# eikehmueller/mlmcpathintegral

Hardware: AMD Instinct MI355X
Metric: lattice-site-updates/sec (higher is better)
Workload: dtype f64

## Files before the change

mlmcpathintegral_amd/csrc/schwinger_perm.hpp:

```cpp
#pragma once
#include "lattice_sweep.hpp"

namespace mlmcpi {

#ifdef MLMCPI_STAMPS
__device__ unsigned long long g_stamps[16 * 65536];
#define MLMCPI_STAMP(k)                                                                                            \
  do {                                                                                                             \
    if (threadIdx.x == 0 && blockIdx.y * gridDim.x + blockIdx.x < 65536)                                           \
      g_stamps[(blockIdx.y * gridDim.x + blockIdx.x) * 16 + (k)] = __builtin_amdgcn_s_memrealtime();               \
  } while (0)
#define MLMCPI_STAMP_WHERE()                                                                                       \
  do {                                                                                                             \
    if (threadIdx.x == 0 && blockIdx.y * gridDim.x + blockIdx.x < 65536)                                           \
      g_stamps[(blockIdx.y * gridDim.x + blockIdx.x) * 16 + 15] =                                                  \
          ((unsigned long long)__builtin_amdgcn_s_getreg((20 ) | (0 << 6) | (31 << 11)) << 32) |         \
          __builtin_amdgcn_s_getreg((4 ) | (0 << 6) | (31 << 11));                                        \
  } while (0)
#else
#define MLMCPI_STAMP(k) do { } while (0)
#define MLMCPI_STAMP_WHERE() do { } while (0)
#endif

#ifndef MLMCPI_PERM_U
#define MLMCPI_PERM_U 0
#endif

template <class PG>
struct PermPlane {
  static constexpr int kRow = PG::kPitch * 8, kStep = kRow + 8;
  static constexpr uint32_t QB = (uint32_t)PG::kQRows * kRow;
  static_assert(kStep == (int)PG::kStep * 8, "the stride of a stream");
  uint32_t K;
  __device__ __forceinline__ explicit PermPlane(uint32_t K_) : K(K_) {}
  __device__ __forceinline__ bool has_col(uint32_t C) const { return (C & 1u) ? C <= PG::col_last(K, 1) : C >= PG::col_first(K, 0) && C <= PG::col_last(K, 0); }
  __device__ __forceinline__ bool has_row(uint32_t R) const { return (R & 1u) ? R <= PG::row_last(K, 1) : R >= PG::row_first(K, 0) && R <= PG::row_last(K, 0); }
  __device__ __forceinline__ uint32_t col(uint32_t C) const { return (C & 1u) ? QB + PG::col_u(K, C) * 8u : PG::col_u(K, C) * 8u; }
  __device__ __forceinline__ uint32_t row(uint32_t R) const { return (R & 1u) ? 2u * QB + PG::row_v(K, R) * (uint32_t)kRow : PG::row_v(K, R) * (uint32_t)kRow; }
};

struct PermBuildPos {
  uint32_t c, r, rend, row_off, gj;
  uint32_t cb;
  const double2 *src;
  uint32_t col;
  bool active, owns;
};
template <int NT, class PP>
__device__ __forceinline__ PermBuildPos perm_build_pos(const PP &P, const double2 *__restrict__ src, uint32_t Mt, uint32_t Mx, uint32_t gi0,
                                                       uint32_t gj0, uint32_t W, uint32_t rows) {
  PermBuildPos q;
  const uint32_t wave = __builtin_amdgcn_readfirstlane(threadIdx.x / kWave), lane = threadIdx.x % kWave;
  const uint32_t nwc = W > 63 ? 2 : 1;
  const uint32_t groups = (NT / kWave) >> (nwc - 1);
  const uint32_t g = wave >> (nwc - 1), cw = wave & (nwc - 1);
  static_assert(((NT / kWave) & (NT / kWave - 1)) == 0, "waves per workgroup: a power of two (shifts for divisions)");
  const uint32_t rpg = groups == 4 ? (rows + 3) >> 2 : groups == 8 ? (rows + 7) >> 3 : (rows + groups - 1) / groups;
  q.c = 63 * cw + lane;
  q.r = __builtin_amdgcn_readfirstlane(g * rpg);
  q.rend = __builtin_amdgcn_readfirstlane(g < groups ? min(rows, q.r + rpg) : 0);
  q.active = q.r < q.rend;
  q.owns = lane < 63 && q.c < W && P.has_col(q.c);
  q.cb = P.col(q.c);
  q.src = src;
  q.col = wrap_add(gi0, min(q.c, W), Mt);
  q.gj = __builtin_amdgcn_readfirstlane(wrap_add(gj0, q.r, Mx));
  q.row_off = q.gj * Mt;
  return q;
}
template <int U>
__device__ __forceinline__ void perm_rows_load(PermBuildPos &q, uint32_t Mt, uint32_t Mx, bool first, double2 &cur, double2 (&nxt)[U]) {
  if (!q.active) return;
  if (first) cur = (q.src + q.row_off)[q.col];
#pragma unroll
  for (int u = 0; u < U; ++u) {
    q.gj = q.gj + 1 == Mx ? 0 : q.gj + 1;
    q.row_off = q.gj == 0 ? 0 : q.row_off + Mt;
    if (q.r + u < q.rend) nxt[u] = (q.src + q.row_off)[q.col];
  }
}
template <int U, class PP>
__device__ __forceinline__ void perm_rows_store(PermBuildPos &q, const PP &P, double *plane, double2 &cur, const double2 (&nxt)[U]) {
  if (!q.active) return;
  char *const pb = reinterpret_cast<char *>(plane) + q.cb;
#pragma unroll
  for (int u = 0; u < U; ++u)
    if (q.r + u < q.rend) {
      const double right = wave_rotate_down(cur.y);
      if (q.owns && P.has_row(q.r + u)) *reinterpret_cast<double *>(pb + P.row(q.r + u)) = ((cur.x + right) - nxt[u].x) - cur.y;
      cur = nxt[u];
    }
  q.r += U;
}
template <int NT, int U, bool ONCE, class PP>
__device__ __forceinline__ void perm_build_rows(const PP &P, double *plane, const double2 *__restrict__ src, uint32_t Mt, uint32_t Mx,
                                                uint32_t gi0, uint32_t gj0, uint32_t W, uint32_t rows) {
  PermBuildPos q = perm_build_pos<NT>(P, src, Mt, Mx, gi0, gj0, W, rows);
  double2 cur = make_double2(0., 0.);
  if (ONCE) {
    double2 nxt[U];
    perm_rows_load<U>(q, Mt, Mx, true, cur, nxt);
    perm_rows_store<U>(q, P, plane, cur, nxt);
    return;
  }
  bool first = true;
  while (__builtin_amdgcn_readfirstlane(q.r) < __builtin_amdgcn_readfirstlane(q.rend)) {
    double2 nxt[U];
    perm_rows_load<U>(q, Mt, Mx, first, cur, nxt);
    perm_rows_store<U>(q, P, plane, cur, nxt);
    first = false;
  }
}

template <int NT, int RING, int TH = 64>
struct PermTasks {
  using PG = PermGeom<NT, RING, TH>;
  static constexpr int OW = PG::OW, HR = PG::HR, H2 = HR / 2, NW = NT / kWave, NS = (HR + NW - 1) / NW;
  static constexpr int XC = OW - 64;
  static constexpr int L0 = XC * H2, L1 = (XC / 2) * HR;
  static constexpr int NL0 = (L0 + 63) / 64, NL1 = (L1 + 63) / 64;
  static constexpr int WF = HR - NW * (NS - 1);
  static_assert(PG::NV == NS, "slots per thread");
  static_assert(NL0 + NL1 <= NW - WF, "the left-over wave-tasks fit the free last slots");
  uint32_t wave, lane, c_mu0, c_mu1, r_lo;
  __device__ PermTasks() {
    wave = __builtin_amdgcn_readfirstlane(threadIdx.x / kWave);
    lane = threadIdx.x % kWave;
    c_mu0 = lane < 32 ? 2 * lane : 2 * (lane - 32) + 1;
    c_mu1 = 2 * (lane & 31u);
    r_lo = lane >> 5;
  }
  __device__ __forceinline__ bool task(int k, bool &mu1, uint32_t &r, uint32_t &c) const {
    const uint32_t m = wave + (uint32_t)(NW * k);
    mu1 = false; r = 0; c = 0;
    if (NW * k + NW - 1 < H2 || m < (uint32_t)H2) {
      r = 2 * m;
      c = c_mu0;
      return true;
    }
    if (m < (uint32_t)HR) {
      mu1 = true;
      r = 2 * (m - H2) + r_lo;
      c = c_mu1;
      return true;
    }
    if (XC > 0 && k == NS - 1) {
      const uint32_t j = wave - (uint32_t)WF;
      if (j < (uint32_t)NL0) {
        const uint32_t L = 64 * j + lane;
        r = 2 * (L / (XC ? XC : 1));
        c = 64 + L % (XC ? XC : 1);
        return L < (uint32_t)L0;
      }
      if (j < (uint32_t)(NL0 + NL1)) {
        const uint32_t L = 64 * (j - NL0) + lane;
        mu1 = true;
        r = L / (XC > 1 ? XC / 2 : 1);
        c = 64 + 2 * (L % (XC > 1 ? XC / 2 : 1));
        return L < (uint32_t)L1;
      }
    }
    return false;
  }
  __device__ __forceinline__ bool valid(int k) const {
    bool mu1; uint32_t r, c;
    return task(k, mu1, r, c);
  }
  __device__ __forceinline__ bool is_mu1(int k) const {
    bool mu1; uint32_t r, c;
    task(k, mu1, r, c);
    return mu1;
  }
  __device__ __forceinline__ void coords(int k, uint32_t &r, uint32_t &c) const {
    bool mu1;
    task(k, mu1, r, c);
  }
};

template <int STEP>
__device__ __forceinline__ void perm_gather5(uint32_t pa, uint32_t px, uint32_t px2, double &S, double &X, double &X2) {
  double a0 = lds_read_f64<0>(pa), x0 = lds_read_f64<0>(px), y0 = lds_read_f64<0>(px2);
  double a1 = lds_read_f64<STEP>(pa), x1 = lds_read_f64<STEP>(px), y1 = lds_read_f64<STEP>(px2);
  double a2 = lds_read_f64<2 * STEP>(pa), x2 = lds_read_f64<2 * STEP>(px), y2 = lds_read_f64<2 * STEP>(px2);
  double a3 = lds_read_f64<3 * STEP>(pa), x3 = lds_read_f64<3 * STEP>(px), y3 = lds_read_f64<3 * STEP>(px2);
  double a4 = lds_read_f64<4 * STEP>(pa), x4 = lds_read_f64<4 * STEP>(px), y4 = lds_read_f64<4 * STEP>(px2);
  asm volatile("s_waitcnt lgkmcnt(0)"
               : "+v"(a0), "+v"(x0), "+v"(y0), "+v"(a1), "+v"(x1), "+v"(y1), "+v"(a2), "+v"(x2), "+v"(y2), "+v"(a3), "+v"(x3), "+v"(y3),
                 "+v"(a4), "+v"(x4), "+v"(y4)
               :
               : "memory");
  S += a0; X += x0; X2 += y0;
  S += a1; X += x1; X2 += y1;
  S += a2; X += x2; X2 += y2;
  S += a3; X += x3; X2 += y3;
  S += a4; X += x4; X2 += y4;
}
__device__ __forceinline__ void perm_gather1(uint32_t pa, uint32_t px, uint32_t px2, double &S, double &X, double &X2) {
  double a0 = lds_read_f64<0>(pa), x0 = lds_read_f64<0>(px), y0 = lds_read_f64<0>(px2);
  asm volatile("s_waitcnt lgkmcnt(0)" : "+v"(a0), "+v"(x0), "+v"(y0) : : "memory");
  S += a0; X += x0; X2 += y0;
}

template <int NT, int RING, int TH = 64>
__device__ __forceinline__ void perm_sweeps(double *plane, const double2 *__restrict__ src, uint32_t Mt, uint32_t Mx, uint32_t i0,
                                            uint32_t j0, uint32_t K, double2 (&res)[2][PermGeom<NT, RING, TH>::NV]) {
  using PG = PermGeom<NT, RING, TH>;
  using PP = PermPlane<PG>;
  constexpr int HR = PG::HR, NV = PG::NV;
  constexpr int kGroups = NT / kWave / 2;
  constexpr int U = MLMCPI_PERM_U ? MLMCPI_PERM_U : (2 * HR + 4 * (int)kPermMaxK + kGroups - 1) / kGroups;
  const uint32_t W = PG::width(K), rows = PG::rows(K), H = RING + 2 * K;
  const PP P(K);
  auto back = [](uint32_t x, uint32_t h, uint32_t n) { return h <= n ? (x >= h ? x - h : x + n - h) : (x + n - h % n) % n; };
  const uint32_t gi0 = back(i0, H, Mt), gj0 = back(j0, H, Mx);
  const uint32_t oi0 = back(i0, RING, Mt), oj0 = back(j0, RING, Mx);
  const PermTasks<NT, RING, TH> tasks;
  const char *const src_b = reinterpret_cast<const char *>(src);
  const bool small_lattice = Mx < (uint32_t)(2 * HR + 2) || Mt < (uint32_t)(PG::OW + 2);
  auto load_theta_of = [&](int h, double2 (&th)[NV], auto small) {
#pragma unroll
    for (int k = 0; k < NV; ++k) {
      if (!tasks.valid(k)) continue;
      uint32_t r, c;
      tasks.coords(k, r, c);
      uint32_t gr = oj0 + r + h * HR, gc = oi0 + c;
      gr = min(gr, gr - Mx);
      gc = min(gc, gc - Mt);
      if ((bool)small) {
        gr = min(gr, gr - Mx); gr = min(gr, gr - Mx);
        gc = min(gc, gc - Mt); gc = min(gc, gc - Mt);
      }
      const uint32_t o = (gr * Mt + gc) * 16u;
      if (!tasks.is_mu1(k)) {
        const uint32_t o2 = gr + 1 == Mx ? o - gr * Mt * 16u : o + Mt * 16u;
        th[k] = make_double2(*reinterpret_cast<const double *>(src_b + o), *reinterpret_cast<const double *>(src_b + o2));
      } else {
        const uint32_t o2 = gc + 1 == Mt ? o - gc * 16u : o + 16u;
        th[k] = make_double2(*reinterpret_cast<const double *>(src_b + o + 8u), *reinterpret_cast<const double *>(src_b + o2 + 8u));
      }
    }
  };
  auto load_theta = [&](int h, double2 (&th)[NV]) {
    if (small_lattice) load_theta_of(h, th, std::true_type{}); else load_theta_of(h, th, std::false_type{});
  };
  auto gather = [&](int h, double2 (&d)[NV]) {
    const uint32_t lds0 = (uint32_t)(uintptr_t)plane;
#pragma unroll
    for (int k = 0; k < NV; ++k) {
      if (!tasks.valid(k)) continue;
      uint32_t r, c;
      tasks.coords(k, r, c);
      const uint32_t ro = r + (uint32_t)(h * HR), cq = c >> 1, rq = ro >> 1;
      uint32_t a, x, x2;
      if (!tasks.is_mu1(k)) {
        const uint32_t cb = (c & 1u) ? PP::QB + ((uint32_t)(PG::OW / 2 - 1) - cq) * 8u : cq * 8u;
        x = cb + rq * (uint32_t)PP::kRow;
        x2 = x + (uint32_t)PP::kRow;
        a = cb + 2u * PP::QB + ((uint32_t)(HR - 1) - rq) * (uint32_t)PP::kRow;
      } else {
        const uint32_t rb = (ro & 1u) ? 2u * PP::QB + ((uint32_t)(HR - 1) - rq) * (uint32_t)PP::kRow : (rq + 1u) * (uint32_t)PP::kRow;
        x = rb + cq * 8u;
        x2 = x + 8u;
        a = rb + PP::QB + ((uint32_t)(PG::OW / 2) - cq) * 8u;
      }
      uint32_t pa = lds0 + a, px = lds0 + x, px2 = lds0 + x2;
      double S = 0.0, X = 0.0, X2 = 0.0;
      uint32_t s = 0;
      for (; s + 5 <= K; s += 5) {
        perm_gather5<PP::kStep>(pa, px, px2, S, X, X2);
        pa += 5 * PP::kStep;
        px += 5 * PP::kStep;
        px2 += 5 * PP::kStep;
      }
      for (; s < K; ++s) {
        perm_gather1(pa, px, px2, S, X, X2);
        pa += PP::kStep;
        px += PP::kStep;
        px2 += PP::kStep;
      }
      d[k] = tasks.is_mu1(k) ? make_double2(X - S, X2 - S) : make_double2(S - X, S - X2);
    }
  };
  auto finish = [&](const double2 (&th)[NV], double2 (&d)[NV]) {
#pragma unroll
    for (int k = 0; k < NV; ++k)
      if (tasks.valid(k)) d[k] = make_double2(mod_2pi_fast(th[k].x + d[k].x), mod_2pi_fast(th[k].y + d[k].y));
  };

  perm_build_rows<NT, U, MLMCPI_PERM_U == 0>(P, plane, src, Mt, Mx, gi0, gj0, W, rows);
  double2 th[NV];
  load_theta(0, th);
  __syncthreads();
  MLMCPI_STAMP(1);
  gather(0, res[0]);
  finish(th, res[0]);
  MLMCPI_STAMP(2);
  load_theta(1, th);
  gather(1, res[1]);
  finish(th, res[1]);
}

template <int NT, int RING, int TH = 64>
__device__ __forceinline__ void perm_store_image(double *th0, double *th1, const double2 (&res)[2][PermGeom<NT, RING, TH>::NV]) {
  using PG = PermGeom<NT, RING, TH>;
  constexpr int OW = PG::OW, HR = PG::HR, NV = PG::NV;
  const PermTasks<NT, RING, TH> tasks;
#pragma unroll
  for (int h = 0; h < 2; ++h)
#pragma unroll
    for (int k = 0; k < NV; ++k) {
      if (!tasks.valid(k)) continue;
      uint32_t r, c;
      tasks.coords(k, r, c);
      const uint32_t o = (r + h * HR) * OW + c;
      if (!tasks.is_mu1(k)) {
        th0[o] = res[h][k].x;
        th0[o + OW] = res[h][k].y;
      } else {
        th1[o] = res[h][k].x;
        th1[o + 1] = res[h][k].y;
      }
    }
}

}
```

Measured before the change: 1057 billion.

## Pair mu0/mu1 tasks per unit and load own theta as double2 with permlane swap

Reorganizes the permutation task mapping so each wave unit handles a row pair for both link directions, with full-wave vector (double2) loads of the owned theta values. The mu1 values are redistributed across lane halves using permlane32_swap instead of separate strided scalar loads. The gather and finish steps are fused into one per-task routine, and the theta loads for the second half are issued split between phases. This aims to cut global load count and improve coalescing, at the cost of extra cross-lane operations and more complex task indexing.

```diff
diff --git a/mlmcpathintegral_amd/csrc/schwinger_perm.hpp b/mlmcpathintegral_amd/csrc/schwinger_perm.hpp
--- a/mlmcpathintegral_amd/csrc/schwinger_perm.hpp
+++ b/mlmcpathintegral_amd/csrc/schwinger_perm.hpp
@@ -115,12 +115,12 @@
 template <int NT, int RING, int TH = 64>
 struct PermTasks {
   using PG = PermGeom<NT, RING, TH>;
-  static constexpr int OW = PG::OW, HR = PG::HR, H2 = HR / 2, NW = NT / kWave, NS = (HR + NW - 1) / NW;
+  static constexpr int OW = PG::OW, HR = PG::HR, H2 = HR / 2, NW = NT / kWave, NS = (HR + NW - 1) / NW, NF = 2 * NS;
   static constexpr int XC = OW - 64;
   static constexpr int L0 = XC * H2, L1 = (XC / 2) * HR;
   static constexpr int NL0 = (L0 + 63) / 64, NL1 = (L1 + 63) / 64;
   static constexpr int WF = HR - NW * (NS - 1);
-  static_assert(PG::NV == NS, "slots per thread");
+  static_assert(PG::NV == NS, "task slots per thread: 2 NV");
   static_assert(NL0 + NL1 <= NW - WF, "the left-over wave-tasks fit the free last slots");
   uint32_t wave, lane, c_mu0, c_mu1, r_lo;
   __device__ PermTasks() {
@@ -130,52 +130,66 @@
     c_mu1 = 2 * (lane & 31u);
     r_lo = lane >> 5;
   }
-  __device__ __forceinline__ bool task(int k, bool &mu1, uint32_t &r, uint32_t &c) const {
-    const uint32_t m = wave + (uint32_t)(NW * k);
-    mu1 = false; r = 0; c = 0;
-    if (NW * k + NW - 1 < H2 || m < (uint32_t)H2) {
-      r = 2 * m;
-      c = c_mu0;
+  __device__ __forceinline__ bool unit(int q, uint32_t &r) const {
+    const uint32_t g = wave + (uint32_t)(NW * q);
+    r = 2 * g;
+    return NW * q + NW - 1 < HR || g < (uint32_t)HR;
+  }
+  __device__ __forceinline__ bool has_unit(int q) const {
+    uint32_t r;
+    return unit(q, r);
+  }
+  __device__ __forceinline__ bool task(int f, bool &mu1, uint32_t &r, uint32_t &c) const {
+    const int q = f >> 1;
+    mu1 = false; c = 0;
+    if (unit(q, r)) {
+      mu1 = f & 1;
+      r += mu1 ? r_lo : 0u;
+      c = mu1 ? c_mu1 : c_mu0;
       return true;
     }
-    if (m < (uint32_t)HR) {
-      mu1 = true;
-      r = 2 * (m - H2) + r_lo;
-      c = c_mu1;
-      return true;
-    }
-    if (XC > 0 && k == NS - 1) {
-      const uint32_t j = wave - (uint32_t)WF;
+    r = 0;
+    if (XC > 0 && q == NS - 1) {
+      const uint32_t j = wave - (uint32_t)WF, r0 = (uint32_t)((f & 1) * HR);
       if (j < (uint32_t)NL0) {
-        const uint32_t L = 64 * j + lane;
-        r = 2 * (L / (XC ? XC : 1));
-        c = 64 + L % (XC ? XC : 1);
+        const uint32_t L = 64 * j + lane, Lc = min(L, (uint32_t)(L0 > 0 ? L0 - 1 : 0));
+        r = r0 + 2 * (Lc / (XC ? XC : 1));
+        c = 64 + Lc % (XC ? XC : 1);
         return L < (uint32_t)L0;
       }
       if (j < (uint32_t)(NL0 + NL1)) {
-        const uint32_t L = 64 * (j - NL0) + lane;
+        const uint32_t L = 64 * (j - NL0) + lane, Lc = min(L, (uint32_t)(L1 > 0 ? L1 - 1 : 0));
         mu1 = true;
-        r = L / (XC > 1 ? XC / 2 : 1);
-        c = 64 + 2 * (L % (XC > 1 ? XC / 2 : 1));
+        r = r0 + Lc / (XC > 1 ? XC / 2 : 1);
+        c = 64 + 2 * (Lc % (XC > 1 ? XC / 2 : 1));
         return L < (uint32_t)L1;
       }
     }
     return false;
   }
-  __device__ __forceinline__ bool valid(int k) const {
+  __device__ __forceinline__ bool left_over(int f) const {
+    return XC > 0 && (f >> 1) == NS - 1 && !has_unit(f >> 1) && wave - (uint32_t)WF < (uint32_t)(NL0 + NL1);
+  }
+  __device__ __forceinline__ bool valid(int f) const {
     bool mu1; uint32_t r, c;
-    return task(k, mu1, r, c);
-  }
-  __device__ __forceinline__ bool is_mu1(int k) const {
+    return task(f, mu1, r, c);
+  }
+  __device__ __forceinline__ bool is_mu1(int f) const {
     bool mu1; uint32_t r, c;
-    task(k, mu1, r, c);
+    task(f, mu1, r, c);
     return mu1;
   }
-  __device__ __forceinline__ void coords(int k, uint32_t &r, uint32_t &c) const {
+  __device__ __forceinline__ void coords(int f, uint32_t &r, uint32_t &c) const {
     bool mu1;
-    task(k, mu1, r, c);
+    task(f, mu1, r, c);
   }
 };
+
+__device__ __forceinline__ double2 own_mu1(double a, double b) {
+  const auto lo = __builtin_amdgcn_permlane32_swap((uint32_t)__double2loint(a), (uint32_t)__double2loint(b), false, false);
+  const auto hi = __builtin_amdgcn_permlane32_swap((uint32_t)__double2hiint(a), (uint32_t)__double2hiint(b), false, false);
+  return make_double2(__hiloint2double((int)hi[0], (int)lo[0]), __hiloint2double((int)hi[1], (int)lo[1]));
+}
 
 template <int STEP>
 __device__ __forceinline__ void perm_gather5(uint32_t pa, uint32_t px, uint32_t px2, double &S, double &X, double &X2) {
@@ -201,12 +215,16 @@
   S += a0; X += x0; X2 += y0;
 }
 
+#ifndef MLMCPI_PERM_NA
+#define MLMCPI_PERM_NA ((NS + 1) / 2)
+#endif
 template <int NT, int RING, int TH = 64>
 __device__ __forceinline__ void perm_sweeps(double *plane, const double2 *__restrict__ src, uint32_t Mt, uint32_t Mx, uint32_t i0,
                                             uint32_t j0, uint32_t K, double2 (&res)[2][PermGeom<NT, RING, TH>::NV]) {
   using PG = PermGeom<NT, RING, TH>;
   using PP = PermPlane<PG>;
-  constexpr int HR = PG::HR, NV = PG::NV;
+  using PT = PermTasks<NT, RING, TH>;
+  constexpr int HR = PG::HR, NV = PG::NV, NS = PT::NS, NF = PT::NF;
   constexpr int kGroups = NT / kWave / 2;
   constexpr int U = MLMCPI_PERM_U ? MLMCPI_PERM_U : (2 * HR + 4 * (int)kPermMaxK + kGroups - 1) / kGroups;
   const uint32_t W = PG::width(K), rows = PG::rows(K), H = RING + 2 * K;
@@ -214,16 +232,33 @@
   auto back = [](uint32_t x, uint32_t h, uint32_t n) { return h <= n ? (x >= h ? x - h : x + n - h) : (x + n - h % n) % n; };
   const uint32_t gi0 = back(i0, H, Mt), gj0 = back(j0, H, Mx);
   const uint32_t oi0 = back(i0, RING, Mt), oj0 = back(j0, RING, Mx);
-  const PermTasks<NT, RING, TH> tasks;
+  const PT tasks;
   const char *const src_b = reinterpret_cast<const char *>(src);
   const bool small_lattice = Mx < (uint32_t)(2 * HR + 2) || Mt < (uint32_t)(PG::OW + 2);
-  auto load_theta_of = [&](int h, double2 (&th)[NV], auto small) {
-#pragma unroll
-    for (int k = 0; k < NV; ++k) {
-      if (!tasks.valid(k)) continue;
+  auto load_own_of = [&](int q0, int q1, double2 (&own)[NS][2], auto small) {
+    uint32_t gc0 = oi0 + tasks.c_mu0;
+    gc0 = min(gc0, gc0 - Mt);
+    if ((bool)small) { gc0 = min(gc0, gc0 - Mt); gc0 = min(gc0, gc0 - Mt); }
+#pragma unroll
+    for (int q = 0; q < NS; ++q) {
+      uint32_t r0;
+      if (q < q0 || q >= q1 || !tasks.unit(q, r0)) continue;
+      uint32_t gr = oj0 + r0;
+      gr = min(gr, gr - Mx);
+      if ((bool)small) { gr = min(gr, gr - Mx); gr = min(gr, gr - Mx); }
+      const uint32_t gr1 = gr + 1 == Mx ? 0 : gr + 1;
+      own[q][0] = *reinterpret_cast<const double2 *>(src_b + (gr * Mt * 16u + gc0 * 16u));
+      own[q][1] = *reinterpret_cast<const double2 *>(src_b + (gr1 * Mt * 16u + gc0 * 16u));
+    }
+  };
+  auto load_left_of = [&](double2 (&lo)[2], auto small) {
+#pragma unroll
+    for (int h = 0; h < 2; ++h) {
+      const int f = NF - 2 + h;
+      if (!tasks.left_over(f)) continue;
       uint32_t r, c;
-      tasks.coords(k, r, c);
-      uint32_t gr = oj0 + r + h * HR, gc = oi0 + c;
+      tasks.coords(f, r, c);
+      uint32_t gr = oj0 + r, gc = oi0 + c;
       gr = min(gr, gr - Mx);
       gc = min(gc, gc - Mt);
       if ((bool)small) {
@@ -231,96 +266,109 @@
         gc = min(gc, gc - Mt); gc = min(gc, gc - Mt);
       }
       const uint32_t o = (gr * Mt + gc) * 16u;
-      if (!tasks.is_mu1(k)) {
+      if (!tasks.is_mu1(f)) {
         const uint32_t o2 = gr + 1 == Mx ? o - gr * Mt * 16u : o + Mt * 16u;
-        th[k] = make_double2(*reinterpret_cast<const double *>(src_b + o), *reinterpret_cast<const double *>(src_b + o2));
+        lo[h] = make_double2(*reinterpret_cast<const double *>(src_b + o), *reinterpret_cast<const double *>(src_b + o2));
       } else {
         const uint32_t o2 = gc + 1 == Mt ? o - gc * 16u : o + 16u;
-        th[k] = make_double2(*reinterpret_cast<const double *>(src_b + o + 8u), *reinterpret_cast<const double *>(src_b + o2 + 8u));
+        lo[h] = make_double2(*reinterpret_cast<const double *>(src_b + o + 8u), *reinterpret_cast<const double *>(src_b + o2 + 8u));
       }
     }
   };
-  auto load_theta = [&](int h, double2 (&th)[NV]) {
-    if (small_lattice) load_theta_of(h, th, std::true_type{}); else load_theta_of(h, th, std::false_type{});
-  };
-  auto gather = [&](int h, double2 (&d)[NV]) {
+  auto load_own = [&](int q0, int q1, double2 (&own)[NS][2]) {
+    if (small_lattice) load_own_of(q0, q1, own, std::true_type{}); else load_own_of(q0, q1, own, std::false_type{});
+  };
+  auto load_left = [&](double2 (&lo)[2]) {
+    if (small_lattice) load_left_of(lo, std::true_type{}); else load_left_of(lo, std::false_type{});
+  };
+  auto one = [&](int f, bool mu1, uint32_t ro, uint32_t c, double2 th) {
     const uint32_t lds0 = (uint32_t)(uintptr_t)plane;
-#pragma unroll
-    for (int k = 0; k < NV; ++k) {
-      if (!tasks.valid(k)) continue;
+    const uint32_t cq = c >> 1, rq = ro >> 1;
+    uint32_t a, x, x2;
+    if (!mu1) {
+      const uint32_t cb = (c & 1u) ? PP::QB + ((uint32_t)(PG::OW / 2 - 1) - cq) * 8u : cq * 8u;
+      x = cb + rq * (uint32_t)PP::kRow;
+      x2 = x + (uint32_t)PP::kRow;
+      a = cb + 2u * PP::QB + ((uint32_t)(HR - 1) - rq) * (uint32_t)PP::kRow;
+    } else {
+      const uint32_t rb = (ro & 1u) ? 2u * PP::QB + ((uint32_t)(HR - 1) - rq) * (uint32_t)PP::kRow : (rq + 1u) * (uint32_t)PP::kRow;
+      x = rb + cq * 8u;
+      x2 = x + 8u;
+      a = rb + PP::QB + ((uint32_t)(PG::OW / 2) - cq) * 8u;
+    }
+    uint32_t pa = lds0 + a, px = lds0 + x, px2 = lds0 + x2;
+    double S = 0.0, X = 0.0, X2 = 0.0;
+    uint32_t s = 0;
+    for (; s + 5 <= K; s += 5) {
+      perm_gather5<PP::kStep>(pa, px, px2, S, X, X2);
+      pa += 5 * PP::kStep;
+      px += 5 * PP::kStep;
+      px2 += 5 * PP::kStep;
+    }
+    for (; s < K; ++s) {
+      perm_gather1(pa, px, px2, S, X, X2);
+      pa += PP::kStep;
+      px += PP::kStep;
+      px2 += PP::kStep;
+    }
+    const double2 d = mu1 ? make_double2(X - S, X2 - S) : make_double2(S - X, S - X2);
+    double2 out = make_double2(mod_2pi_fast(th.x + d.x), mod_2pi_fast(th.y + d.y));
+    asm volatile("" : "+v"(out.x), "+v"(out.y));
+    res[f / NV][f % NV] = out;
+  };
+  auto gather = [&](int q0, int q1, const double2 (&own)[NS][2]) {
+#pragma unroll
+    for (int q = 0; q < NS; ++q) {
+      uint32_t r0;
+      if (q < q0 || q >= q1 || !tasks.unit(q, r0)) continue;
+      one(2 * q, false, r0, tasks.c_mu0, make_double2(own[q][0].x, own[q][1].x));
+      one(2 * q + 1, true, r0 + tasks.r_lo, tasks.c_mu1, own_mu1(own[q][0].y, own[q][1].y));
+    }
+  };
+  auto gather_left = [&](const double2 (&lo)[2]) {
+#pragma unroll
+    for (int h = 0; h < 2; ++h) {
+      const int f = NF - 2 + h;
+      if (!tasks.left_over(f)) continue;
       uint32_t r, c;
-      tasks.coords(k, r, c);
-      const uint32_t ro = r + (uint32_t)(h * HR), cq = c >> 1, rq = ro >> 1;
-      uint32_t a, x, x2;
-      if (!tasks.is_mu1(k)) {
-        const uint32_t cb = (c & 1u) ? PP::QB + ((uint32_t)(PG::OW / 2 - 1) - cq) * 8u : cq * 8u;
-        x = cb + rq * (uint32_t)PP::kRow;
-        x2 = x + (uint32_t)PP::kRow;
-        a = cb + 2u * PP::QB + ((uint32_t)(HR - 1) - rq) * (uint32_t)PP::kRow;
-      } else {
-        const uint32_t rb = (ro & 1u) ? 2u * PP::QB + ((uint32_t)(HR - 1) - rq) * (uint32_t)PP::kRow : (rq + 1u) * (uint32_t)PP::kRow;
-        x = rb + cq * 8u;
-        x2 = x + 8u;
-        a = rb + PP::QB + ((uint32_t)(PG::OW / 2) - cq) * 8u;
-      }
-      uint32_t pa = lds0 + a, px = lds0 + x, px2 = lds0 + x2;
-      double S = 0.0, X = 0.0, X2 = 0.0;
-      uint32_t s = 0;
-      for (; s + 5 <= K; s += 5) {
-        perm_gather5<PP::kStep>(pa, px, px2, S, X, X2);
-        pa += 5 * PP::kStep;
-        px += 5 * PP::kStep;
-        px2 += 5 * PP::kStep;
-      }
-      for (; s < K; ++s) {
-        perm_gather1(pa, px, px2, S, X, X2);
-        pa += PP::kStep;
-        px += PP::kStep;
-        px2 += PP::kStep;
-      }
-      d[k] = tasks.is_mu1(k) ? make_double2(X - S, X2 - S) : make_double2(S - X, S - X2);
-    }
-  };
-  auto finish = [&](const double2 (&th)[NV], double2 (&d)[NV]) {
-#pragma unroll
-    for (int k = 0; k < NV; ++k)
-      if (tasks.valid(k)) d[k] = make_double2(mod_2pi_fast(th[k].x + d[k].x), mod_2pi_fast(th[k].y + d[k].y));
+      tasks.coords(f, r, c);
+      one(f, tasks.is_mu1(f), r, c, lo[h]);
+    }
   };
 
   perm_build_rows<NT, U, MLMCPI_PERM_U == 0>(P, plane, src, Mt, Mx, gi0, gj0, W, rows);
-  double2 th[NV];
-  load_theta(0, th);
+  constexpr int NA = MLMCPI_PERM_NA;
+  double2 own[NS][2], lo[2];
+  load_own(0, NA, own);
   __syncthreads();
   MLMCPI_STAMP(1);
-  gather(0, res[0]);
-  finish(th, res[0]);
+  gather(0, NA, own);
   MLMCPI_STAMP(2);
-  load_theta(1, th);
-  gather(1, res[1]);
-  finish(th, res[1]);
+  load_own(NA, NS, own);
+  if (PT::XC > 0) load_left(lo);
+  gather(NA, NS, own);
+  if (PT::XC > 0) gather_left(lo);
 }
 
 template <int NT, int RING, int TH = 64>
 __device__ __forceinline__ void perm_store_image(double *th0, double *th1, const double2 (&res)[2][PermGeom<NT, RING, TH>::NV]) {
   using PG = PermGeom<NT, RING, TH>;
-  constexpr int OW = PG::OW, HR = PG::HR, NV = PG::NV;
+  constexpr int OW = PG::OW, NV = PG::NV;
   const PermTasks<NT, RING, TH> tasks;
 #pragma unroll
-  for (int h = 0; h < 2; ++h)
-#pragma unroll
-    for (int k = 0; k < NV; ++k) {
-      if (!tasks.valid(k)) continue;
-      uint32_t r, c;
-      tasks.coords(k, r, c);
-      const uint32_t o = (r + h * HR) * OW + c;
-      if (!tasks.is_mu1(k)) {
-        th0[o] = res[h][k].x;
-        th0[o + OW] = res[h][k].y;
-      } else {
-        th1[o] = res[h][k].x;
-        th1[o + 1] = res[h][k].y;
-      }
-    }
-}
-
-}
+  for (int f = 0; f < 2 * NV; ++f) {
+    if (!tasks.valid(f)) continue;
+    uint32_t r, c;
+    tasks.coords(f, r, c);
+    const uint32_t o = r * OW + c;
+    if (!tasks.is_mu1(f)) {
+      th0[o] = res[f / NV][f % NV].x;
+      th0[o + OW] = res[f / NV][f % NV].y;
+    } else {
+      th1[o] = res[f / NV][f % NV].x;
+      th1[o + 1] = res[f / NV][f % NV].y;
+    }
+  }
+}
+
+}
```

Result: no change. 1064 billion (median of 6 runs) (+0.7%).
